# seungju-k1m/sac-td3-td7

Hardware: AMD Instinct MI355X
Metric: gradient-steps/sec (whole node), TD7 Humanoid-v4 batch=256 at 1/2/4/8 GPUs (higher is better)
Workload: dtype fp32

## Files before the change

### include/rle.h

```cpp
#ifndef RLE_H
#define RLE_H

#ifdef __cplusplus
extern "C" {
#endif

#define RLE_TD7 0
#define RLE_TD3 1
#define RLE_SAC 2

#define RLE_INFO_MAX 8

#define RLE_OK 0
#define RLE_EINVAL (-1)
#define RLE_EHIP (-2)
#define RLE_ESTATE (-3)

typedef struct rle_replay rle_replay;
typedef struct rle_engine rle_engine;

typedef struct rle_config {
  int algo;
  int state_dim, action_dim;
  int hidden;
  int batch;
  int use_lap;
  float discount;
  float policy_lr, critic_lr;
  float tau;
  float target_policy_noise, noise_clip;
  int policy_freq;
  int target_update_rate;
  float min_log_std, max_log_std;
  float tmp;
  unsigned long long seed;
  int device;
  int zs_dim;
  int n_hidden;
  int hidden_sizes[8];
  int act_actor, act_critic, act_encoder;
  float bc_lambda;
} rle_config;
typedef struct rle_config_ext {
  int size;
  float bc_alpha;
} rle_config_ext;
#define RLE_MAX_HIDDEN 6
#define RLE_ACT_DEFAULT 0
#define RLE_ACT_RELU 1
#define RLE_ACT_ELU 2
#define RLE_ACT_IDENTITY 3
#define RLE_ACT_LEAKY_RELU 4
#define RLE_ACT_SILU 5
#define RLE_ACT_GELU 6

#define RLE_FUSE_PRELAYER (1u << 0)
#define RLE_FUSE_PRE      (1u << 1)
#define RLE_FUSE_QDOT     (1u << 2)
#define RLE_FUSE_HEADDX   (1u << 3)
#define RLE_FUSE_NBDEFER  (1u << 4)
#define RLE_FUSE_SACFWD   (1u << 5)
#define RLE_FUSE_SACBWD   (1u << 6)
#define RLE_FUSE_FOLD     (1u << 7)
#define RLE_FUSE_PIPOLYAK (1u << 8)
#define RLE_FUSE_ENDSPLIT (1u << 9)
#define RLE_FUSE_PRIOSAMPLE (1u << 10)
#define RLE_FUSE_TWOSTAGE (1u << 11)
#define RLE_FUSE_SACPRE   (1u << 12)
#define RLE_FUSE_NORMFIN  (1u << 13)
#define RLE_FUSE_OPT_IN RLE_FUSE_PRIOSAMPLE
typedef struct rle_plan {
  int level_cap;
  int steps_per_graph;
  int pre_tn;
  int pl_tn;
  int tn_min;
  int flat_div;
  int balance;
  int tiny_w, uni_w, tiny_wg;
  int sched_cap;
  unsigned fuse_off;
  unsigned fuse_on;
  int rb;
  int pl_w;
  int lap_w, head_w, adam_w;
  int wide;
  int lpt;
  int dispatch;
  int dpf;
  int xcd;
} rle_plan;


int rle_replay_create(int device, long long capacity, int state_dim, int action_dim, int lap,
                      rle_replay** out);
int rle_replay_destroy(rle_replay* r);
int rle_replay_append(rle_replay* r, const float* state, const float* action, const float* reward,
                      const float* next_state, const float* notdone, long long count);
int rle_replay_state(rle_replay* r, long long* ptr, long long* size, float* max_priority);
int rle_replay_fill_random(rle_replay* r, long long count, unsigned long long seed);
int rle_replay_get_priority(rle_replay* r, float* out, long long n);
int rle_replay_set_priority(rle_replay* r, const float* p, long long n, float max_priority);
int rle_replay_sample_indices(rle_replay* r, int n, const float* u, long long* ind_out);
int rle_replay_update_priority(rle_replay* r, int n, const long long* ind, const float* p);
int rle_replay_reset_max_priority(rle_replay* r);
int rle_replay_gather(rle_replay* r, int n, const long long* ind, float* state, float* action,
                      float* reward, float* next_state, float* notdone);
int rle_replay_io_rows(void);
int rle_replay_export(rle_replay* r, long long first, long long count, float* state, float* action,
                      float* reward, float* next_state, float* notdone, float* priority);
int rle_replay_import(rle_replay* r, long long first, long long count, const float* state,
                      const float* action, const float* reward, const float* next_state,
                      const float* notdone, const float* priority);
int rle_replay_set_state(rle_replay* r, long long ptr, long long size, float max_priority);
int rle_replay_copy(rle_replay* dst, rle_replay* src);
int rle_replay_state_stats(rle_replay* r, float* mean, float* std);
int rle_replay_normalize_states(rle_replay* r, const float* shift, const float* scale);


int rle_create(const rle_config* cfg, rle_engine** out);
int rle_create_ext(const rle_config* cfg, const rle_config_ext* ext, rle_engine** out);
int rle_destroy(rle_engine* e);
// ... 67 lines not shown
```

### sac-td3-td7_amd/csrc/engine.cpp

```cpp
#include <hip/hip_runtime.h>
#include <hsa/hsa.h>
#include <hsa/hsa_ext_amd.h>
#include <hsa/hsa_ven_amd_loader.h>

#include <algorithm>
#include <atomic>
#include <chrono>
#include <cstdlib>
#include <cmath>
#include <cstdio>
#include <cstring>
#include <map>
#include <memory>
#include <mutex>
#include <stdexcept>
#include <string>
#include <thread>
#include <vector>

#include "ops.h"
#include "rle.h"

namespace rle {
hipError_t launch_level(const Op* d_ops, const Op* h_ops, int nops, int nwg, hipStream_t st,
// ... 233 lines not shown
  return 64;
}

static void check_gemm(const GemmArgs& g) {
  auto chk = [&](const Operand& o, bool xsplit, int xn) {
    REQUIRE(o.nseg >= 1 && o.nseg <= kMaxSeg, "gemm: bad segment count");
    for (int q = 0; q < o.nseg; ++q) {
      const Seg& s = o.seg[q];
      REQUIRE(s.p != nullptr && s.r0 % 16 == 0 && s.r1 > s.r0, "gemm: bad reduction segment");
      if (!xsplit) {
        REQUIRE(s.x0 == 0 && s.x1 >= xn, "gemm: segment must span the operand rows");
        if (q) REQUIRE(s.r0 == r16(o.seg[q - 1].r1), "gemm: reduction segments must be back to back");
      } else {
        REQUIRE(s.x0 % 16 == 0 && s.x1 % 16 == 0 && s.r0 == o.seg[0].r0 && s.r1 == o.seg[0].r1,
                "gemm: bad column split");
      }
    }
  };
  chk(g.A, false, g.M);
  chk(g.B, g.mode == GEMM_DW, g.N);
  if (g.mode == GEMM_DX || (g.mode == GEMM_FWD && g.B.nseg > 1)) {
    REQUIRE(g.B.nseg == g.A.nseg, "gemm: one W segment per A segment");
    for (int q = 0; q < g.A.nseg; ++q)
      REQUIRE(g.B.seg[q].r0 == g.A.seg[q].r0 && g.B.seg[q].r1 == g.A.seg[q].r1, "gemm: W / A segment mismatch");
  }
  REQUIRE(g.R <= 16 * 1024, "gemm: reduction too long");
}

static void xcd_plan(GemmArgs& g, bool xcd);

static bool gemm_variant_compiled(int vid, int ks = -1) {
#define RLE_VID(mode, epi, act, norm, pre, pk, sets) \
  (vid == gemm_vid(mode, epi, act, norm, pre) && (ks < 0 || ks_family(ks) == KS_EXT || (((sets) >> ks_family(ks)) & 1))) ||
  return RLE_GEMM_VARIANTS(RLE_VID) false;
#undef RLE_VID
}

static void gemm_finalize(GemmArgs& g, bool xcd = true) {
  int norm = 0;
  for (int q = 0; q < g.A.nseg; ++q) norm |= g.A.seg[q].norm.part != nullptr;
  for (int q = 0; q < g.B.nseg; ++q) norm |= g.B.seg[q].norm.part != nullptr;
  const int act_rt = g.mode == GEMM_FWD ? g.act : (g.mode == GEMM_DX ? g.dact : ACT_NONE);
  const int act = g.mode == GEMM_DW ? g.act : act_vslot(act_rt);
  REQUIRE(act_rt >= ACT_NONE && act_rt <= ACT_GELU, "gemm: activation");
  REQUIRE(act_rt <= ACT_TANH || ((g.has_pre == 0 || g.has_pre == 2) &&
                                 (g.epi == EPI_STORE || g.epi == EPI_QDOT || g.epi == EPI_QHEAD)),
          "gemm: LeakyReLU / SiLU / GELU run the plain and fused-loss-head paths only (kernels.hip kActRt)");
  REQUIRE(g.mode != GEMM_DX || !norm, "gemm: no DX variant with normed operands");
  REQUIRE(g.mode != GEMM_DW || g.epi == EPI_ADAM, "gemm: DW is always fused with Adam");
  REQUIRE(g.mode != GEMM_DW || act == ACT_NONE || (act == kDwGs && !norm && g.gscale) ||
              (act == kDwNb && !norm && g.nbx.t && g.nbm.part && g.nbdot && g.R <= 1024),
          "gemm: deferred AvgL1Norm backward / gradient scale operands");
  REQUIRE(g.mode != GEMM_DW || (act == kDwGs) == (g.gscale != nullptr), "gemm: gscale is the kDwGs variant's");
  REQUIRE(g.epi != EPI_NBDOT || (g.mode == GEMM_DX && act == ACT_NONE && g.nbx.t && g.norm_out),
          "gemm: EPI_NBDOT is a plain DX with x and partials");
  REQUIRE(g.epi != EPI_MSE || act == ACT_NONE, "gemm: MSE epilogue takes no activation");
  REQUIRE((g.dact == ACT_NONE) == (g.dsrc.t == nullptr) || g.mode != GEMM_DX, "gemm: DX derivative source");
  REQUIRE(g.has_pre != 1 || ((g.mode == GEMM_FWD || g.mode == GEMM_DX) && g.prea.N <= 32 && g.prea.seg < g.A.nseg &&
                               g.A.seg[g.prea.seg].r1 - g.A.seg[g.prea.seg].r0 <= 32 && g.prea.mode == g.mode &&
                               g.prea.R % 16 == 0),
          "gemm: pre-GEMM layout");
  {
    const HeadArgs& h = g.hd;
    const bool pol = h.mode == HEAD_MLP_POLICY;
    const bool modes = (h.mode == HEAD_TD7_LOSS && h.tgt_mode == HEAD_TD7_TARGET && h.vt && h.vmax_key && h.vmin_key) ||
                       (h.mode == HEAD_MLP_LOSS && h.tgt_mode == HEAD_MLP_TARGET && !h.vt) ||
                       (pol && h.tgt_mode < 0 && !h.lap && h.tp_n[0] == 0 && h.tp_n[1] == 0);
    const bool parts = h.qp[0] && h.qp[1] && h.qp_n[0] <= 64 && h.qp_n[1] <= 64 &&
                       (pol || (h.tp[0] && h.tp[1] && h.tp_n[0] <= 64 && h.tp_n[1] <= 64));
    REQUIRE(g.has_pre != 2 || (g.mode == GEMM_DX && g.epi == EPI_STORE && (act == ACT_ELU || act == ACT_RELU) &&
                               !norm && g.A.nseg == 1 && modes && parts && h.dact == act_rt && (!h.sac || h.logpi) &&
                               (!h.lap || h.prio) && h.H <= 256 && h.H % 4 == 0 && g.R == r16(h.H) &&
                               g.M % 16 == 0 && h.rows == h.nvalid && h.rows <= g.M && g.M - h.rows < 16 &&
                               (g.head_n == 0 || g.head_n == 1)),
            "gemm: fused loss head layout");
  }
  REQUIRE(g.epi != EPI_SACFWD || (g.mode == GEMM_FWD && act == ACT_NONE && !norm && g.has_pre == 0 && g.tn == 64 &&
                                   g.tiles_n == 1 && g.sf.A <= 32 && g.sf.ls_off + g.sf.A <= g.N && g.sf.eps.t &&
                                   g.sf.eps2.t && (g.sf.act.n || g.sf.act.t) && g.sf.logpi),
          "gemm: SAC actor forward epilogue operands");
  REQUIRE(g.epi != EPI_SACBWD || (g.mode == GEMM_DX && act == ACT_NONE && !norm && g.has_pre == 0 && g.sb.raw.t &&
                                   g.sb.eps2.t && (g.sb.dout.n || g.sb.dout.t) && g.sb.log_alpha &&
                                   g.sb.ls_off >= g.sb.mean_off + g.N),
          "gemm: SAC actor backward epilogue operands");
  REQUIRE((g.has_pre != 3 && g.has_pre != 4) || (((g.mode == GEMM_FWD && (g.epi == EPI_STORE || g.epi == EPI_QDOT) && g.prea.bias) ||
                                (g.mode == GEMM_DX && g.epi == EPI_STORE && g.prea.dsrc.t)) &&
                               act == ACT_RELU && !norm && g.A.nseg == 1 && g.prea.seg == 0 && g.prea.mode == g.mode &&
                               g.prea.act == ACT_RELU && g.prea.N == g.A.seg[0].r1 - g.A.seg[0].r0 && g.prea.N <= 256 &&
                               g.prea.N % 16 == 0 && g.prea.R % 16 == 0 && g.prea.R <= 48 && g.prea.B.nseg == 1 &&
                               g.R == g.prea.N &&
                               !g.pre.t && g.B.nseg == 1),
          "gemm: pre-layer layout");
  {
    const PreArgs& q = g.prea2;
    REQUIRE(g.has_pre != 4 || (g.mode == GEMM_FWD && g.epi == EPI_QDOT && q.mode == GEMM_FWD && q.N <= 32 &&
                               q.R % 16 == 0 && q.R <= 16 * 1024 && q.A.nseg == 1 && q.B.nseg == 1 &&
                               q.seg == 1 && g.prea.A.nseg == 2 && g.prea.A.seg[0].r0 == 0 &&
                               g.prea.A.seg[q.seg].r1 - g.prea.A.seg[q.seg].r0 <= 16 &&
                               g.prea.A.seg[q.seg].r0 % 16 == 0),
            "gemm: two-stage pre-layer layout");
  }
  {
    const PreArgs& q = g.prea;
    REQUIRE(g.has_pre != 5 || (g.mode == GEMM_FWD && g.epi == EPI_STORE && act == ACT_RELU && !norm &&
                               q.mode == GEMM_FWD && q.A.nseg == 1 && q.B.nseg == 1 && q.sac_a >= 1 &&
                               q.N == 2 * q.sac_a && q.N <= 48 && q.R % 16 == 0 && q.R <= 256 && q.bias &&
// ... 680 lines not shown
      const std::string what = a.what ? a.what : "";
      if (what.rfind("tape", 0) == 0) continue;
      const bool in_p = a.lo >= p0 && a.hi <= p1;
      if (!a.w || what == "adam w.t" || what == "adam bias") {
        if (op.kind == OP_GEMM && a.t >= 0) xr[(op.wg_begin + a.t) & 7].push_back({a.lo, a.hi});
        else once.push_back({a.lo, a.hi});
      }
      if (what.rfind("adam", 0) == 0) {
        if (a.w) t.adam_w += (double)(a.hi - a.lo);
        ad.push_back({a.lo, a.hi});
        if (what == "adam w.t" || what == "adam bias") ad.push_back({a.lo, a.hi});
      } else if (a.w) {
        aw.push_back({a.lo, a.hi});
      } else if (in_p) {
        wr.push_back({a.lo, a.hi});
      } else {
        ar.push_back({a.lo, a.hi});
      }
    }
  }
  t.act_r += union_bytes(ar);
  t.act_w += union_bytes(aw);
  t.w_r += union_bytes(wr);
  double adam = 0;
  for (auto& r : ad) adam += (double)(r.second - r.first);
  t.adam = adam;
  double xb = union_bytes(once);
  for (auto& r : xr) xb += union_bytes(r);
  t.xcd_r = xb;
  return t;
}

struct Prog {
  struct Item {
    std::vector<Op> ops;
    std::vector<int> rd, wr;
    int level = 0;
  };
  std::vector<Item> items;
  static constexpr int max_ops = kLevelOps;
  int rb = 0;
  int xcd = 1;
  std::map<const float*, std::pair<float*, int>> norm_fins;
  static bool rb_eligible(const GemmArgs& g) {
    bool seg_ok = true;
    for (int q = 0; q < g.B.nseg; ++q) seg_ok = seg_ok && g.B.seg[q].x0 % g.tn == 0;
    return g.mode == GEMM_DW && (g.tn == 32 || g.tn == 64) && g.has_pre == 0 && seg_ok;
  }
  void add(const Op& op, std::vector<int> rd, std::vector<int> wr) { add_group({op}, std::move(rd), std::move(wr)); }
  void add_group(std::vector<Op> ops, std::vector<int> rd, std::vector<int> wr) {
    for (Op& op : ops)
      if (op.kind == OP_GEMM) {
        op.gemm.hot.rb = rb && rb_eligible(op.gemm) ? 1 : 0;
        gemm_finalize(op.gemm, xcd != 0);
        check_gemm(op.gemm);
        if (std::getenv("RLE_AUDIT")) audit_gemm(op.gemm);
      }
    Item it;
    it.ops = std::move(ops);
    it.rd = std::move(rd);
    it.wr = std::move(wr);
    items.push_back(std::move(it));
  }
  int balance = 0;
  int tiny_w = 30, uni_w = 60, tiny_wg = 2;
  int pl_w = 0;
  int lap_w = 60, head_w = 60, adam_w = 8;
  int lpt = 0;
  int tiny_weight() const { return tiny_w ? tiny_w : 8; }
  int uniform_weight() const { return uni_w; }
  bool tiny_moves() const { return tiny_w != 0; }
  int op_weight(const Op& op) const {
    int x = 8;
    if (op.kind == OP_GEMM)
      x = op.gemm.R * op.gemm.tn / 1024 + (op.gemm.epi == EPI_ADAM ? adam_w : 0) + (op.gemm.has_pre >= 3 ? pl_w : 0);
    else if (op.kind == OP_HEAD) x = head_w;
    else if (op.kind == OP_SAMPLE_GATHER) x = op.sample.lap ? lap_w : uniform_weight();
    else if (op.kind == OP_STEP_END && op.end.mode != 1) x = tiny_weight();
    return x;
  }
  int item_weight(const Item& it) const {
    int w = 0;
    for (const Op& op : it.ops) w = std::max(w, op_weight(op));
    return w;
  }
  std::vector<std::vector<int>> successors() const {
    const int n = (int)items.size();
    std::vector<std::vector<int>> succ(n);
    std::map<int, int> lastw;
    std::map<int, std::vector<int>> readers;
    for (int i = 0; i < n; ++i) {
      const Item& it = items[i];
      auto edge = [&](int from) {
        if (from >= 0) succ[from].push_back(i);
      };
      for (int r : it.rd)
        if (r >= 0 && lastw.count(r)) edge(lastw[r]);
      for (int w : it.wr) {
        if (w < 0) continue;
        if (lastw.count(w)) edge(lastw[w]);
        for (int j : readers[w]) edge(j);
      }
      for (int w : it.wr)
        if (w >= 0) {
          lastw[w] = i;
          readers[w].clear();
// ... 1517 lines not shown
    g.A.seg[0] = seg_t(dz, 0, 0, Brows);
    g.A.nseg = 1;
    int koff = 0;
    for (size_t s = 0; s < X.size(); ++s) {
      const View& v = X[s];
      REQUIRE(v.cols == L.seg_p[s] && v.rows >= Brows && v.m.t, "dw: input view mismatch for " + L.wname);
      g.B.seg[s] = seg_t(v, koff, 0, Brows);
      if (v.norm && fused(RLE_FUSE_NORMFIN)) {
        const auto f = norm_fin(pg, v);
        g.B.seg[s].norm = f.first;
        rd.push_back(f.second);
      } else if (v.norm) {
        rd.push_back(v.norm_id);
      }
      rd.push_back(v.id);
      koff += L.seg_p[s];
    }
    g.B.nseg = (int)X.size();
    g.M = L.out;
    g.N = L.K;
    g.R = Brows;
    const auto tq = choose_tn(L.out, L.K);
    g.tn = tq.first;
    op.seq = tq.second;
    g.tiles_m = cdiv(L.out, kTileM);
    g.tiles_n = cdiv(L.K, g.tn) + 1;
    g.epi = EPI_ADAM;
    AdamArgs& ad = g.adam;
    ad.w = wmat(L);
    ad.b = bias(L);
    ad.mo = (long long)nP;
    ad.vo = 2LL * (long long)nP;
    ad.step = adam_step_of(asc_set) + cnt;
    ad.bc2s = adam_bc2s_of(asc_set) + cnt;
    ad.lr = lr;
    ad.beta1 = 0.9f;
    g.gscale = o.gscale;
    if (o.gscale) {
      REQUIRE(!nb_x, "dw: no gradient scale with a deferred AvgL1Norm backward");
      g.act = kDwGs;
      rd.push_back(o.gscale_id);
    }
    ad.beta2 = 0.999f;
    ad.omb1 = (float)(1.0 - 0.9);
    ad.omb2 = (float)(1.0 - 0.999);
    ad.eps = 1e-8f;
    ad.bias_col = cdiv(L.K, g.tn) * g.tn;
    ad.gsq = o.gsq;
    ad.gsq_b = o.gsq_b;
    ad.ptau = o.ptau;
    if (nb_x) {
      REQUIRE(dz.nbdot && nb_x->norm && nb_x->m.t && nb_x->rows >= Brows, "dw: deferred AvgL1Norm backward operands");
      g.act = kDwNb;
      g.nbx = nb_x->m;
      g.nbx_xs = nb_x->m.rbs;
      g.nbm = nb_x->nref();
      g.nbdot = dz.nbdot;
      g.nbdot_ld = dz.nbdot_ld;
      g.nbdot_n = dz.nbdot_n;
      rd.push_back(nb_x->id);
      if (fused(RLE_FUSE_NORMFIN)) {
        const auto f = norm_fin(pg, *nb_x);
        g.nbm = f.first;
        g.nb_width = nb_x->width;
        rd.push_back(f.second);
      } else {
        rd.push_back(nb_x->norm_id);
      }
      rd.push_back(dz.nbdot_id);
    }
    op.wg_count = g.tiles_m * g.tiles_n;
    pg.add(op, rd, wr);
  }

  bool pi_polyak_fused() const { return fused(RLE_FUSE_PIPOLYAK); }

  std::pair<NormRef, int> norm_fin(Prog& pg, const View& v) {
    REQUIRE(v.norm && v.norm_ld > 0, "norm_fin: not a normed view");
    auto it = pg.norm_fins.find(v.norm);
    if (it == pg.norm_fins.end()) {
      Op op{};
      op.kind = OP_NORMBWD;
      NormBwdArgs& a = op.nb;
      a.fwd = 2;
      a.rows = v.norm_ld;
      a.width = v.width;
      a.norm.part = v.norm;
      a.norm.ld = v.norm_ld;
      a.norm.row0 = 0;
      a.norm.nparts = v.nparts;
      a.norm.width = v.width;
      a.mout = mem.make<float>((size_t)v.norm_ld);
      op.wg_count = cdiv(v.norm_ld, kThreads);
      const int id = next_id++;
      pg.add(op, {v.norm_id}, {id});
      it = pg.norm_fins.emplace(v.norm, std::make_pair(a.mout, id)).first;
    }
    NormRef r{};
    r.part = it->second.first;
    r.ld = v.norm_ld;
    r.row0 = v.norm_row0;
    r.nparts = 1;
    r.width = 1;
    return {r, it->second.second};
  }

// ... 1208 lines not shown
  Graph capture(Prog& pg) {
    pg.balance = plan.balance;
    pg.tiny_w = plan.tiny_w;
    pg.uni_w = plan.uni_w;
    pg.tiny_wg = plan.tiny_wg;
    pg.pl_w = plan.pl_w;
    pg.lap_w = plan.lap_w;
    pg.head_w = plan.head_w;
    pg.adam_w = plan.adam_w;
    pg.lpt = plan.lpt;
    auto levels = pg.schedule(sched_cap());
    Graph G;
    size_t total = 0;
    for (auto& lv : levels) {
      G.nlaunch += (int)((lv.size() + kLevelOps - 1) / kLevelOps);
      G.off.push_back((int)total);
      G.nops.push_back((int)lv.size());
      int wg = 0;
      for (auto& op : lv) wg += op.wg_count;
      G.nwg.push_back(wg);
      total += lv.size();
    }
    static const char* kname[] = {"?", "gemm", "normbwd", "sreduce", "sgather", "head", "prio",
                                  "sacfwd", "sacbwd", "end", "polyak", "copy", "maxred", "ctrl", "noise",
                                  "foldbias", "bc"};
    static const bool traffic = [] {
      const char* e = std::getenv("RLE_TRAFFIC");
      return e && e[0] == '1';
    }();
    for (size_t l = 0; l < levels.size(); ++l) {
      G.desc += "L" + std::to_string(l) + " wg=" + std::to_string(G.nwg[l]) + ":";
      if (traffic) {
        const LevelTraffic t = level_traffic(levels[l], P, nP);
        char buf[220];
        snprintf(buf, sizeof buf, " [KB act_r %.0f act_w %.0f w_r %.0f adam %.0f other %.0f xcd_r %.0f adam_w %.0f]",
                 t.act_r / 1024, t.act_w / 1024, t.w_r / 1024, t.adam / 1024, t.other / 1024, t.xcd_r / 1024,
                 t.adam_w / 1024);
        G.desc += buf;
      }
      for (size_t k = 0; k < levels[l].size(); ++k) {
        const Op& op = levels[l][k];
        G.desc += std::string(" ") + (pg.crit_lv[l][k] ? "*" : "") + kname[op.kind];
        if (op.kind == OP_GEMM) {
          static const char* kepi[] = {"st", "adam", "mse", "qhead", "nbdot", "act", "qdot", "sacbwd", "sacfwd"};
          static_assert(sizeof(kepi) / sizeof(kepi[0]) == EPI_SACFWD + 1, "every epilogue has a name");
          const char* ep = op.gemm.mode == GEMM_DW && op.gemm.act == kDwNb ? "adam+nb"
                           : op.gemm.mode == GEMM_DW && op.gemm.act == kDwGs ? "adam+gs"
                           : op.gemm.has_pre == 2                         ? "head+dx"
                           : op.gemm.has_pre == 3                         ? (op.gemm.epi == EPI_QDOT ? "qdot+pl" : "st+pl")
                           : op.gemm.has_pre == 4                         ? "qdot+pl2"
                           : op.gemm.has_pre == 5                         ? "st+sacpre"
                                                                           : kepi[op.gemm.epi];
          G.desc += "[" + std::to_string(op.gemm.M) + "x" + std::to_string(op.gemm.N) + "x" +
                    std::to_string(op.gemm.R) + " " + ep + (op.gemm.hot.wide ? ".w" : "");
          const int art = op.gemm.mode == GEMM_FWD ? op.gemm.act : op.gemm.mode == GEMM_DX ? op.gemm.dact : ACT_NONE;
          if (art > ACT_TANH) G.desc += art == ACT_LEAKY ? " leaky" : art == ACT_SILU ? " silu" : " gelu";
          G.desc += "]";
        }
        if (std::getenv("RLE_DESC_WG")) G.desc += "/" + std::to_string(op.wg_count);
      }
      G.desc += "\n";
    }
    std::vector<Op> flat_ops;
    flat_ops.reserve(total);
    for (auto& lv : levels)
      for (auto& op : lv) {
        REQUIRE(op.kind != OP_GEMM || gemm_variant_compiled(op.gemm.vid, kernel_set()),
                "capture: a GEMM variant outside the engine's rle_level instance (ops.h RLE_GEMM_VARIANTS sets)");
        REQUIRE(kernel_set() == KS_ACT ||
                    ((op.kind != OP_GEMM || op.gemm.mode == GEMM_DW ||
                      (op.gemm.mode == GEMM_FWD ? op.gemm.act : op.gemm.dact) <= ACT_TANH) &&
                     (op.kind != OP_HEAD || op.head.dact <= ACT_TANH)),
                "capture: an activation of the KS_ACT rle_level instance in another instance's program");
        flat_ops.push_back(op);
      }
    G.d_ops = mem.make<Op>(total);
    HIPCHK(hipMemcpy(G.d_ops, flat_ops.data(), total * sizeof(Op), hipMemcpyHostToDevice));
    const char* tr_env = std::getenv("RLE_TRACE");
    if (tr_env && tr_env[0] == '1') {
      for (int w : G.nwg) G.trace_n += w;
      G.trace = mem.make<unsigned long long>((size_t)G.trace_n * trace_stride());
    }
    if (plan.dispatch == 1 && !G.trace) g_level_rec = &G.aql;
    HIPCHK(hipStreamBeginCapture(stream, hipStreamCaptureModeThreadLocal));
    long long tr_off = 0;
    const bool dpf = plan.dpf != 0;
    for (size_t l = 0; l < levels.size(); ++l) {
      const size_t ln = l + 1 < levels.size() ? l + 1 : 0;
      hipError_t e = launch_level(G.d_ops + G.off[l], levels[l].data(), G.nops[l], G.nwg[l], stream,
                                  G.trace ? G.trace + tr_off * trace_stride() : nullptr, G.d_ops + G.off[ln],
                                  dpf ? G.nops[ln] : 0, kernel_set());
      tr_off += G.nwg[l];
      if (e != hipSuccess) {
        g_level_rec = nullptr;
        hipGraph_t tmp;
        (void)hipStreamEndCapture(stream, &tmp);
        throw Error{RLE_EHIP, std::string("launch during capture: ") + hipGetErrorString(e)};
      }
    }
    g_level_rec = nullptr;
    HIPCHK(hipStreamEndCapture(stream, &G.g));
    if (!G.aql.empty()) {
      std::vector<unsigned char> ka(G.aql.size() * 128, 0);
      for (size_t i = 0; i < G.aql.size(); ++i) std::memcpy(ka.data() + i * 128, G.aql[i].ka, sizeof G.aql[i].ka);
      G.aql_ka = mem.make<unsigned char>(ka.size());
      HIPCHK(hipMemcpy(G.aql_ka, ka.data(), ka.size(), hipMemcpyHostToDevice));
    }
// ... 1763 lines not shown
```

### sac-td3-td7_amd/csrc/kernels.hip

```cpp
#include <hip/hip_runtime.h>
#include <math.h>
#include <stdint.h>

#include <cstring>
#include <type_traits>
#include <vector>

#include "ops.h"

#define CAS __attribute__((address_space(4)))
#define GAS __attribute__((address_space(1)))

namespace rle {

typedef float f32x4 __attribute__((ext_vector_type(4)));

template <class T>
__device__ __forceinline__ const GAS T* G(const T* p) {
  return (const GAS T*)p;
}
template <class T>
__device__ __forceinline__ GAS T* GW(T* p) {
  return (GAS T*)p;
}
// ... 402 lines not shown
      x[r] = bload(rx, vx + nx * 1024);
      if (!bias_ones) b[r] = bload(rb, vb + nx * 1024);
    }
  }
  return acc + acc1;
}

template <int RPT, int PM, int PD>
__device__ __forceinline__ void nb_tab_batched(const CAS GemmArgs& g, int n, float* ti, float* tg, float xw, int r0 = 0) {
  float sm[RPT], sd[RPT];
  row_sums<RPT, PM>(g.nbm.part, g.nbm.ld, g.nbm.row0 + r0, g.nbm.nparts, n, sm);
  row_sums<RPT, PD>(g.nbdot, g.nbdot_ld, r0, g.nbdot_n, n, sd);
#pragma unroll
  for (int r = 0; r < RPT; ++r) {
    const int i = threadIdx.x + r * kThreads;
    const float mean = sm[r] / (float)g.nbm.width, dot = sd[r] / 1.f;
    const bool clamped = mean < 1e-8f;
    const float inv = 1.f / (clamped ? 1e-8f : mean);
    if (i < n) {
      ti[i] = inv;
      tg[i] = clamped ? 0.f : (-dot * inv * inv) / xw;
    }
  }
}
__device__ __forceinline__ void build_nb_tab(const CAS GemmArgs& g, int n, float* ti, float* tg) {
  const float xw = (float)(g.nb_width ? g.nb_width : g.nbm.width);
  const int pm = g.nbm.nparts, pd = g.nbdot_n;
  if (n <= kThreads && pm <= 16 && pd <= 16) {
    nb_tab_batched<1, 16, 16>(g, n, ti, tg, xw);
    return;
  }
  if (n <= 4 * kThreads && pm == 1 && pd <= 8) {
    nb_tab_batched<4, 1, 8>(g, n, ti, tg, xw);
    return;
  }
  if (n <= 4 * kThreads && pm <= 4 && pd <= 4) {
    nb_tab_batched<4, 4, 4>(g, n, ti, tg, xw);
    return;
  }
  if (n <= 4 * kThreads && pm == 1 && pd <= 16) {
    nb_tab_batched<2, 1, 16>(g, min(n, 2 * kThreads), ti, tg, xw);
    if (n > 2 * kThreads) nb_tab_batched<2, 1, 16>(g, n - 2 * kThreads, ti + 2 * kThreads, tg + 2 * kThreads, xw, 2 * kThreads);
    return;
  }
#pragma unroll 1
  for (int i = threadIdx.x; i < n; i += kThreads) {
    const float mean = norm_mean_i(g.nbm.part, g.nbm.ld, i + g.nbm.row0, g.nbm.nparts, g.nbm.width);
    const float dot = norm_mean_i(g.nbdot, g.nbdot_ld, i, g.nbdot_n, 1);
    const bool clamped = mean < 1e-8f;
    const float inv = 1.f / (clamped ? 1e-8f : mean);
    ti[i] = inv;
    tg[i] = clamped ? 0.f : (-dot * inv * inv) / xw;
  }
}

__device__ __forceinline__ void chunk_loop2(__amdgpu_buffer_rsrc_t ra, int va, __amdgpu_buffer_rsrc_t rb, int vb0,
                                            int vb1, int n, f32x4& acc0, f32x4& acc1) {
  float4 a[kRing], b0[kRing], b1[kRing];
#pragma unroll
  for (int r = 0; r < kRing; ++r) {
    if (r >= n) break;
    a[r] = bload(ra, va + r * 1024);
    b0[r] = bload(rb, vb0 + r * 1024);
    b1[r] = bload(rb, vb1 + r * 1024);
  }
#pragma unroll 1
  for (int c = 0; c < n; c += kRing) {
#pragma unroll
    for (int r = 0; r < kRing; ++r) {
      if (c + r >= n) break;
      acc0 = mfma4(a[r], b0[r], acc0);
      acc1 = mfma4(a[r], b1[r], acc1);
      const int nx = c + r + kRing;
      if (nx >= n) continue;
      a[r] = bload(ra, va + nx * 1024);
      b0[r] = bload(rb, vb0 + nx * 1024);
      b1[r] = bload(rb, vb1 + nx * 1024);
    }
  }
}

constexpr int kRbOff = 2048;
template <int NB, int RG>
struct RbRing {
  float4 a[RG], x[RG], b[RG][NB];
};
template <int NB, int RG, bool NBX>
__device__ __forceinline__ void rb_issue(RbRing<NB, RG>& R, __amdgpu_buffer_rsrc_t ra, int va,
                                         __amdgpu_buffer_rsrc_t rbr, const int (&vbv)[NB], int nb, int n,
                                         __amdgpu_buffer_rsrc_t rx, int vx, bool bias_ones) {
  const float4 ones = make_float4(1.f, 1.f, 1.f, 1.f);
#pragma unroll
  for (int r = 0; r < RG; ++r) {
    if (r >= n) break;
    R.a[r] = bload(ra, va + r * 1024);
    if constexpr (NBX) R.x[r] = bload(rx, vx + r * 1024);
#pragma unroll
    for (int cb = 0; cb < NB; ++cb)
      if (cb < nb) R.b[r][cb] = bias_ones ? ones : bload(rbr, vbv[cb] + r * 1024);
  }
}
template <int NB, int RG, bool NBX>
__device__ __forceinline__ void rb_run(RbRing<NB, RG>& R, __amdgpu_buffer_rsrc_t ra, int va,
                                       __amdgpu_buffer_rsrc_t rbr, const int (&vbv)[NB], int nb, int n,
                                       f32x4 (&acc)[NB], const float* tabb, __amdgpu_buffer_rsrc_t rx, int vx,
                                       const float* ti, const float* tg, bool bias_ones) {
// ... 1062 lines not shown
      constexpr bool NBX = ACT == kDwNb;
      const int nq = (nch + 3) >> 2, q0 = wave * nq, q1 = min(nch, q0 + nq), nrun = max(0, q1 - q0);
      const int jc0 = jt * tn;
      int nb = 0;
#pragma unroll
      for (int cb = 0; cb < NB; ++cb) nb = jc0 + cb * 16 < gN ? cb + 1 : nb;
      if (bias_tile) nb = 1;
      int qb = 0;
#pragma unroll
      for (int q = 1; q < kMaxSeg; ++q)
        if (q < nseg_b && min(jc0, gN - 1) >= g.B.seg[q].x0) qb = q;
      const CAS Seg& sbq = g.B.seg[qb];
      int vbv[NB];
#pragma unroll
      for (int cb = 0; cb < NB; ++cb) vbv[cb] = ((((jc0 - sbq.x0) >> 4) + cb) * sbq.xs + q0) * 1024 + lb;
      const int va = ((i0 >> 4) * a0xs + q0) * 1024 + lb;
      const int vx = NBX ? ((i0 >> 4) * g.nbx_xs + q0) * 1024 + lb : 0;
      const auto rx = NBX ? rsrc(g.nbx.t) : rsrc(a0p);
      RbRing<NB, RG> R;
      rb_issue<NB, RG, NBX>(R, rsrc(a0p), va, rsrc(sbq.p), vbv, nb, nrun, rx, vx, bias_tile);
      const float* tabb = nullptr;
      if constexpr (NORM) {
        if (sbq.norm.part) build_norm_tab(sbq.norm, sbq.r1 - sbq.r0, tabs);
        __syncthreads();
        if (sbq.norm.part && !bias_tile) tabb = tabs + q0 * 16;
      }
      int tgo = 0;
      if constexpr (NBX) {
        tgo = (gR + 15) & ~15;
        build_nb_tab(g, gR, tabs, tabs + tgo);
        __syncthreads();
      }
      f32x4 ac[NB];
#pragma unroll
      for (int cb = 0; cb < NB; ++cb) ac[cb] = f32x4{0.f, 0.f, 0.f, 0.f};
      rb_run<NB, RG, NBX>(R, rsrc(a0p), va, rsrc(sbq.p), vbv, nb, nrun, ac, tabb, rx, vx, tabs + q0 * 16,
                          tabs + tgo + q0 * 16, bias_tile);
      acc = rb_exchange<NB>(ac, smem, cg, lead);
    };
    if (tn == 64) rbw(std::integral_constant<int, 4>{});
    else rbw(std::integral_constant<int, 2>{});
  } else {
    int qb = 0;
#pragma unroll
    for (int q = 1; q < kMaxSeg; ++q)
      if (q < nseg_b && j0 >= g.B.seg[q].x0) qb = q;
    const CAS Seg& sb = g.B.seg[qb];
    const bool run = active && c0 < c1;
    const int va = ((i0 >> 4) * a0xs + c0) * 1024 + lb;
    const int vb = (((j0 - sb.x0) >> 4) * sb.xs + c0) * 1024 + lb;
    const int vx = ACT == kDwNb ? ((i0 >> 4) * g.nbx_xs + c0) * 1024 + lb : 0;
    const int nrun = run ? c1 - c0 : 0;
    constexpr int RGD = ACT == kDwNb ? kRing : kRingDW;
    float4 ra[RGD], rb[RGD], rx[RGD];
    ring_issue<RGD>(ra, rb, rsrc(a0p), va, rsrc(sb.p), vb, nrun, bias_tile);
    if constexpr (ACT == kDwNb) {
#pragma unroll
      for (int r = 0; r < RGD; ++r)
        if (r < nrun) rx[r] = bload(rsrc(g.nbx.t), vx + r * 1024);
    }
    FINE_MARK(0);
    const float* tb = nullptr;
    if constexpr (NORM) {
      int off = 0, mine = -1;
      for (int q = 0; q < nseg_b; ++q) {
        const CAS Seg& s = g.B.seg[q];
        if (!s.norm.part) continue;
        build_norm_tab(s.norm, s.r1 - s.r0, tabs + off);
        if (q == qb) mine = off;
        off += (s.r1 - s.r0 + 15) & ~15;
      }
      __syncthreads();
      if (mine >= 0) tb = tabs + mine + c0 * 16;
    }
    int tgo = 0;
    if constexpr (ACT == kDwNb) {
      tgo = (gR + 15) & ~15;
      build_nb_tab(g, gR, tabs, tabs + tgo);
      __syncthreads();
    }
    FINE_MARK(1);
    if (run) {
      if constexpr (ACT == kDwNb) {
        acc = ring_run_nb<RGD>(ra, rx, rb, rsrc(a0p), va, rsrc(g.nbx.t), vx, rsrc(sb.p), vb, nrun, acc,
                               tabs + c0 * 16, tabs + tgo + c0 * 16, bias_tile);
      } else if (NORM && tb && !bias_tile)
        acc = ring_run<0, 2, RGD>(ra, rb, rsrc(a0p), va, rsrc(sb.p), vb, nrun, acc, 1.f, nullptr, tb, bias_tile);
      else
        acc = ring_run<0, 0, RGD>(ra, rb, rsrc(a0p), va, rsrc(sb.p), vb, nrun, acc, 1.f, nullptr, nullptr, bias_tile);
    }
  }
  trace_mark(tr, 2);
  if (ksl && !rbm) {
    if (!lead) *(f32x4*)(part + (wave * 64 + lane) * 4) = acc;
    __syncthreads();
    if (lead) {
      for (int q = 1; q < (1 << ksl); ++q) acc += *(const f32x4*)(part + ((wave + q) * 64 + lane) * 4);
    }
  }
  FINE_MARK(9);

  if constexpr (EPI == EPI_STORE || EPI == EPI_QDOT) {
    auto epi_store = [&](const f32x4 acc, const int i0, const int ib, const float4 ds, float* red) {
      float rowabs[4] = {0.f, 0.f, 0.f, 0.f};
      if (jok) {
        float y[4];
#pragma unroll
        for (int q = 0; q < 4; ++q) y[q] = acc[q] + pre_b;
        if constexpr (MODE == GEMM_FWD) {
          if (g.pre.t) mat_st4(g.pre, ib, j, make_float4(y[0], y[1], y[2], y[3]));
#pragma unroll
          for (int q = 0; q < 4; ++q) y[q] = act_f<ACT>(y[q], g.act);
          if constexpr (ACT == ACT_TANH) {
            if (g.noise.t && ib >= g.noise_row0) {
              const float4 e = mat_ld4(g.noise, ib - g.noise_row0, j);
              const float ev[4] = {e.x, e.y, e.z, e.w};
#pragma unroll
              for (int q = 0; q < 4; ++q) {
                const float nz = fminf(fmaxf(ev[q] * g.noise_sigma, -g.noise_clip), g.noise_clip);
                y[q] = fminf(fmaxf(y[q] + nz, -1.f), 1.f);
              }
            }
          }
        } else {
          const float dv[4] = {ds.x, ds.y, ds.z, ds.w};
#pragma unroll
          for (int q = 0; q < 4; ++q) y[q] *= act_b<ACT>(dv[q], g.dact);
        }
#pragma unroll
        for (int q = 0; q < 4; ++q) rowabs[q] = EPI == EPI_QDOT ? y[q] * qwj : fabsf(y[q]);
        mat_st4(g.out, ib, j, make_float4(y[0], y[1], y[2], y[3]));
      }
      if constexpr (MODE == GEMM_FWD) {
        if (EPI == EPI_QDOT || g.norm_out) {
#pragma unroll
// ... 1119 lines not shown
      d2 += d * d;
      GW(b.e.n)[nidx(b.e.cbn, r, j)] = c * d;
    }
    d2 = wg_sum(d2, smem);
    if (tid == 0) GW(b.part)[t] = d2;
    return;
  }
  if (BC3 && b.mode == 2) {
    float sa = 0.f;
    for (int i = tid; i < b.qp_n[0]; i += kThreads) sa += G(b.qp[0])[(size_t)i * b.qp_ld];
    const float q_abs = wg_sum(sa, smem) / (float)B;
    if (tid == 0) {
      GW(b.out)[0] = q_abs;
      GW(b.out)[1] = b.lambda / q_abs;
    }
    if (tid < A) GW(b.eye.t)[tidx(b.eye.rbs, tid, tid)] = q_abs / b.lambda;
    return;
  }
  const float b0 = G(b.qb[0])[0], b1 = G(b.qb[1])[0];
  float qa = 0.f;
  for (int r = tid; r < B; r += kThreads) {
    const float q0 = norm_mean_i(b.qp[0], b.qp_ld, r, b.qp_n[0], 1);
    const float q1 = norm_mean_i(b.qp[1], b.qp_ld, r, b.qp_n[1], 1);
    qa += BC3 && b.mode == 3 ? fabsf(fminf(q0 + b0, q1 + b1)) : fabsf(q0 + b0) + fabsf(q1 + b1);
  }
  if (BC3 && b.mode == 3) {
    const float q_abs = wg_sum(qa, smem) / (float)B;
    if (tid == 0) {
      GW(b.out)[0] = q_abs;
      GW(b.out)[1] = b.lambda / q_abs;
    }
    if (tid < A) GW(b.eye.t)[tidx(b.eye.rbs, tid, tid)] = q_abs / b.lambda;
    return;
  }
  const float q_abs = wg_sum(qa, smem) / (2.f * (float)B);
  if (tid == 0) GW(b.out)[0] = q_abs;
  if (tid < A) GW(b.eye.t)[tidx(b.eye.rbs, tid, tid)] = q_abs;
}


static_assert(kLevelOps == 12, "rle_level takes the op table as 12 scalar arguments");

template <bool TRACE, int KS>
#ifndef RLE_WAVES
#define RLE_WAVES 4
#endif
__global__ __launch_bounds__(kThreads, RLE_WAVES) void rle_level(unsigned e0, unsigned e1, unsigned e2, unsigned e3,
                                                                  unsigned e4, unsigned e5, unsigned e6, unsigned e7,
                                                                  unsigned e8, unsigned e9, unsigned e10, unsigned e11,
                                                                  const Op* ops_arg, unsigned long long* trace_arg,
                                                                  const Op* next_arg, unsigned next_lines) {
  constexpr int kSmemF = (KS == KS_TD7W || ks_family(KS) == KS_EXT) && kWideSmem > 6144 ? kWideSmem : 6144;
  static_assert(kSmemF >= kRbOff + 4096, "LDS for the register-blocked exchange");
  __shared__ __attribute__((aligned(16))) float smem[kSmemF];
  const unsigned long long t_in = TRACE ? __builtin_amdgcn_s_memrealtime() : 0ull;
  if ((e0 >> 31) && blockIdx.x < 8) {
    const unsigned nl = next_lines;
    const char* nb = (const char*)next_arg;
    unsigned v0 = 0, v1 = 0;
    const unsigned l0 = threadIdx.x, l1 = threadIdx.x + kThreads;
    if (l0 < nl) asm volatile("global_load_dword %0, %1, off" : "=v"(v0) : "v"(nb + l0 * 64) : "memory");
    if (l1 < nl) asm volatile("global_load_dword %0, %1, off" : "=v"(v1) : "v"(nb + l1 * 64) : "memory");
    asm volatile("s_waitcnt vmcnt(0)" ::"v"(v0), "v"(v1) : "memory");
    return;
  }
  const unsigned entry[kLevelOps] = {e0 & 0x7fffffffu, e1, e2, e3, e4, e5, e6, e7, e8, e9, e10, e11};
  const int wg = (int)blockIdx.x - (int)(e0 >> 31) * 8;
  int k = 0;
  unsigned e = entry[0];
#pragma unroll
  for (int q = 1; q < kLevelOps; ++q) {
    const unsigned x = entry[q];
    const bool in = (int)(x & 0xffffu) <= wg;
    e = in ? x : e;
    k = in ? q : k;
  }
  const int kind = (e >> 16) & 0xf, vid = e >> 20;
  const CAS Op* ops = (const CAS Op*)ops_arg;
  const int wb = (int)(e & 0xffffu);
  const CAS Op& op = ops[k];
  const int t = wg - wb;
  unsigned long long* tr = TRACE ? trace_arg + (size_t)wg * kTraceStride : nullptr;
  if (TRACE && threadIdx.x == 0) tr[0] = t_in;
  if (kind != OP_GEMM) {
    unsigned dsink;
    asm volatile(
        "s_load_dword %0, %1, 0x0\n\t"
        "s_load_dword %0, %1, 0x40\n\t"
        "s_load_dword %0, %1, 0x80\n\t"
        "s_load_dword %0, %1, 0xc0\n\t"
        "s_load_dword %0, %1, 0x100\n\t"
        "s_load_dword %0, %1, 0x140\n\t"
        "s_load_dword %0, %1, 0x180\n\t"
        "s_load_dword %0, %1, 0x1c0\n\t"
        "s_waitcnt lgkmcnt(0)"
        : "=&s"(dsink)
        : "s"(&op));
    (void)dsink;
  }
  FINE_MARK(7);
  switch (kind) {
#define RLE_OP(K, call)                       \
  case K:                                     \
    asm volatile("; op case " #K ::);         \
    call;                                     \
    break;
// ... 599 lines not shown
```

### sac-td3-td7_amd/csrc/ops.h

```cpp
#pragma once
#include <stdint.h>

namespace rle {

constexpr int kThreads = 256;
constexpr int kTileM = 16;
constexpr int kTileN = 64;
constexpr int kMaxSeg = 4;
constexpr int kInfoMax = 8;
constexpr int kMaxHidden = 6;
constexpr int kGsqT = 2 * (kMaxHidden + 1);

enum OpKind : int {
  OP_GEMM = 1,
  OP_NORMBWD = 2,
  OP_SAMPLE_REDUCE = 3,
  OP_SAMPLE_GATHER = 4,
  OP_HEAD = 5,
  OP_PRIORITY = 6,
  OP_SAC_ACTOR = 7,
  OP_SAC_ACTOR_BWD = 8,
  OP_STEP_END = 9,
  OP_POLYAK = 10,
  OP_COPY = 11,
// ... 94 lines not shown
  X(GEMM_FWD, EPI_MSE, ACT_NONE, 1, 0, 0, 1)        \
  X(GEMM_FWD, EPI_ACT, ACT_TANH, 0, 0, 0, 3)        \
  X(GEMM_FWD, EPI_QDOT, ACT_ELU, 0, 0, 0, 1)        \
  X(GEMM_FWD, EPI_QDOT, ACT_RELU, 0, 0, 0, 2)       \
  X(GEMM_FWD, EPI_QDOT, ACT_NONE, 0, 0, 0, 0)       \
  X(GEMM_DX, EPI_STORE, ACT_NONE, 0, 0, 0, 3)       \
  X(GEMM_DX, EPI_STORE, ACT_RELU, 0, 0, 0, 3)       \
  X(GEMM_DX, EPI_STORE, ACT_ELU, 0, 0, 0, 3)        \
  X(GEMM_DX, EPI_STORE, ACT_TANH, 0, 0, 0, 3)       \
  X(GEMM_DX, EPI_NBDOT, ACT_NONE, 0, 0, 0, 1)       \
  X(GEMM_DW, EPI_ADAM, ACT_NONE, 0, 0, 0, 3)        \
  X(GEMM_DW, EPI_ADAM, ACT_NONE, 1, 0, 0, 1)        \
  X(GEMM_DW, EPI_ADAM, kDwNb, 0, 0, 0, 1)           \
  X(GEMM_DW, EPI_ADAM, kDwGs, 0, 0, 0, 0)           \
  X(GEMM_FWD, EPI_STORE, ACT_NONE, 0, 1, 1, 1)      \
  X(GEMM_FWD, EPI_STORE, ACT_RELU, 0, 1, 1, 3)      \
  X(GEMM_FWD, EPI_STORE, ACT_ELU, 1, 1, 1, 1)       \
  X(GEMM_DX, EPI_STORE, ACT_RELU, 0, 1, 1, 3)       \
  X(GEMM_DX, EPI_SACBWD, ACT_NONE, 0, 0, 0, 2)      \
  X(GEMM_FWD, EPI_SACFWD, ACT_NONE, 0, 0, 0, 2)     \
  X(GEMM_DX, EPI_STORE, ACT_ELU, 0, 2, 2, 1)        \
  X(GEMM_DX, EPI_STORE, ACT_RELU, 0, 2, 2, 2)       \
  X(GEMM_FWD, EPI_STORE, ACT_RELU, 0, 3, 3, 2)      \
  X(GEMM_FWD, EPI_QDOT, ACT_RELU, 0, 3, 3, 2)       \
  X(GEMM_DX, EPI_STORE, ACT_RELU, 0, 3, 3, 2)       \
  X(GEMM_FWD, EPI_QDOT, ACT_RELU, 1, 3, 4, 2)       \
  X(GEMM_FWD, EPI_STORE, ACT_RELU, 1, 1, 5, 2)
constexpr bool wide_variant(int mode, int epi, int pk) {
  return pk == 0 && mode != 2  &&
         (epi == EPI_STORE || epi == EPI_QDOT || epi == EPI_MSE || epi == EPI_QHEAD || epi == EPI_NBDOT);
}
enum KernelSet : int { KS_TD7 = 0, KS_MLP = 1, KS_EXT = 2, KS_TD7W = 3, KS_ACT = 4, KS_COUNT = 5 };
constexpr int ks_family(int ks) { return ks == KS_TD7W ? KS_TD7 : ks == KS_ACT ? KS_EXT : ks; }

enum GemmMode : int {
  GEMM_FWD = 0,
  GEMM_DX = 1,
  GEMM_DW = 2,
};

struct GemmHot {
  int ks_log, tiles_n, tn, N, R;
  float inv_tiles_n;
  int bias_col, nseg_a, nseg_b;
  int a0xs, a0r0, a0r1, b0xs, tiles;
  const float* a0p;
  const float* b0p;
  const float* bias;
  int xb, tmb;
  float inv_tmb, inv_xb, inv_blast;
  int nfull;
  int rb;
  int wide;
  int pad_[4];
};
static_assert(sizeof(GemmHot) == 128, "GemmHot is loaded as 2 x 16 dwords");

__host__ __device__ inline void xcd_tile(int t, int T, int tiles_n, int xb, int tmb, int nfull, float inv_tmb,
                                         float inv_xb, float inv_blast, int& it, int& jt) {
  const int q = T >> 3, m = T & 7, r0 = t & 7;
  const int p = r0 * q + (r0 < m ? r0 : m) + (t >> 3);
  const int band = (int)(((float)p + 0.5f) * inv_tmb);
  const int rem = p - band * tmb;
  const bool full = band < nfull;
  const int bw = full ? xb : tiles_n - nfull * xb;
  it = (int)(((float)rem + 0.5f) * (full ? inv_xb : inv_blast));
  jt = band * xb + rem - it * bw;
}

struct PreArgs {
  Operand A, B;
  int mode;
  int N, R;
  int seg;
  int act;
  int sac_a;
  const float* bias;
  Mat noise; float noise_sigma, noise_clip;
  Mat dsrc;
};

enum HeadMode : int {
  HEAD_TD7_TARGET = 0,
  HEAD_TD7_LOSS = 1,
  HEAD_TD7_POLICY = 2,
  HEAD_MLP_TARGET = 3,
  HEAD_MLP_LOSS = 4,
  HEAD_MLP_POLICY = 5,
};

struct HeadArgs {
  int mode, rows, H, lap;
  Mat h[2];
  Mat dsrc[2];
  int dact;
  int nvalid;
  const float* w[2];
  int w_cbn;
  const float* b[2];
  const float* reward; const float* notdone;
  float* y;
  Mat dz[2];
  Mat dq[2];
  float* loss_part;
  float* prio;
  float gamma;
  int sac;
  int alpha_lin;
  const float* logpi;
// ... 362 lines not shown
```

### sac-td3-td7_amd/rl/_engine.py

```python

from __future__ import annotations

import contextlib
import ctypes
import os
import threading

import numpy as np

RLE_TD7, RLE_TD3, RLE_SAC = 0, 1, 2
RLE_EVAL_Q, RLE_EVAL_ZS, RLE_EVAL_ZSA = 0, 1, 2
INFO_MAX = 8
REPLAY_IO_ROWS = 8192

_HERE = os.path.dirname(os.path.abspath(__file__))
LIB_PATH = os.environ.get("RLE_LIB") or os.path.join(os.path.dirname(_HERE), "lib", "librle.so")

_lib = None

_f32p = ctypes.POINTER(ctypes.c_float)
_i64p = ctypes.POINTER(ctypes.c_longlong)
_vp = ctypes.c_void_p
_cs = ctypes.c_char_p
_int = ctypes.c_int
_ll = ctypes.c_longlong


class Config(ctypes.Structure):

    _fields_ = [
        ("algo", _int), ("state_dim", _int), ("action_dim", _int), ("hidden", _int),
        ("batch", _int), ("use_lap", _int), ("discount", ctypes.c_float),
        ("policy_lr", ctypes.c_float), ("critic_lr", ctypes.c_float), ("tau", ctypes.c_float),
        ("target_policy_noise", ctypes.c_float), ("noise_clip", ctypes.c_float),
        ("policy_freq", _int), ("target_update_rate", _int), ("min_log_std", ctypes.c_float),
        ("max_log_std", ctypes.c_float), ("tmp", ctypes.c_float), ("seed", ctypes.c_ulonglong),
        ("device", _int), ("zs_dim", _int), ("n_hidden", _int), ("hidden_sizes", _int * 8),
        ("act_actor", _int), ("act_critic", _int), ("act_encoder", _int),
        ("bc_lambda", ctypes.c_float),
    ]


class ConfigExt(ctypes.Structure):

    _fields_ = [("size", _int), ("bc_alpha", ctypes.c_float)]


def make_config_ext(bc_alpha=0.0) -> ConfigExt:
    return ConfigExt(ctypes.sizeof(ConfigExt), float(bc_alpha))


ACT_CODES = {"default": 0, "relu": 1, "elu": 2, "identity": 3, "leaky_relu": 4, "silu": 5, "gelu": 6}


class Plan(ctypes.Structure):

    _fields_ = [
        ("level_cap", _int), ("steps_per_graph", _int), ("pre_tn", _int), ("pl_tn", _int), ("tn_min", _int),
        ("flat_div", _int), ("balance", _int), ("tiny_w", _int), ("uni_w", _int), ("tiny_wg", _int),
        ("sched_cap", _int), ("fuse_off", ctypes.c_uint), ("fuse_on", ctypes.c_uint), ("rb", _int),
        ("pl_w", _int), ("lap_w", _int), ("head_w", _int), ("adam_w", _int), ("wide", _int), ("lpt", _int),
        ("dispatch", _int), ("dpf", _int), ("xcd", _int),
    ]


FUSE = {"prelayer": 1 << 0, "pre": 1 << 1, "qdot": 1 << 2, "headdx": 1 << 3, "nbdefer": 1 << 4, "sacfwd": 1 << 5,
        "sacbwd": 1 << 6, "fold": 1 << 7, "pipolyak": 1 << 8, "endsplit": 1 << 9, "priosample": 1 << 10,
        "twostage": 1 << 11, "sacpre": 1 << 12, "normfin": 1 << 13}


def make_plan(fuse_off=(), fuse_on=(), **kw) -> Plan:
    p = Plan()
    _check(lib().rle_plan_default(ctypes.byref(p)))
    for k, v in kw.items():
        if k not in dict(Plan._fields_):
            raise ValueError(f"unknown plan field {k!r}")
        setattr(p, k, int(v))
    def bits(names):
        b = 0
        for name in ([names] if isinstance(names, str) else names):
            b |= FUSE[name]
        return b

    p.fuse_off, p.fuse_on = bits(fuse_off), bits(fuse_on)
    return p


def parse_plan(text: str) -> Plan:
    kw, off, on = {}, (), ()
    for item in filter(None, (t.strip() for t in (text or "").split(","))):
        k, _, v = item.partition("=")
        if k == "fuse_off":
            off = tuple(filter(None, v.split("+")))
        elif k == "fuse_on":
            on = tuple(filter(None, v.split("+")))
        else:
            kw[k] = int(v)
    return make_plan(off, on, **kw)


def plan_dict(p: Plan) -> dict:
    d = {k: getattr(p, k) for k, _ in Plan._fields_}
    d["fuse_off"] = [n for n, b in FUSE.items() if p.fuse_off & b]
    d["fuse_on"] = [n for n, b in FUSE.items() if p.fuse_on & b]
    return d


STATE_PARAMS, STATE_ADAM_M, STATE_ADAM_V, STATE_ALL = 1, 2, 4, 7

_scratch = np.empty(0, np.float32)
_scratch_lock = threading.Lock()


@contextlib.contextmanager
def state_scratch(n):
    global _scratch
    with _scratch_lock:
        if _scratch.size < n:
            _scratch = np.empty(n, np.float32)
        yield _scratch[:n]

# ... 489 lines not shown
```

Before: 8330.

## Stage AvgL1Norm-backward strip in LDS for kDwNb weight-gradient GEMMs

Adds a staged path for the deferred AvgL1Norm-backward weight-gradient GEMM. Each wave computes a share of the normalized-gradient rows and writes them into a shared LDS strip, then after a barrier all waves run MFMAs from that strip. Previously each wave recomputed the transform from its own global loads. The path is gated by a new fuse bit and by an LDS-fit check on R. It keeps per-element fused/unfused FMA ordering so results stay bitwise identical, at the cost of an added block barrier and LDS traffic.

```diff
diff --git a/include/rle.h b/include/rle.h
--- a/include/rle.h
+++ b/include/rle.h
@@ -68,6 +68,7 @@
 #define RLE_FUSE_TWOSTAGE (1u << 11)
 #define RLE_FUSE_SACPRE   (1u << 12)
 #define RLE_FUSE_NORMFIN  (1u << 13)
+#define RLE_FUSE_NBSTAGE  (1u << 14)
 #define RLE_FUSE_OPT_IN RLE_FUSE_PRIOSAMPLE
 typedef struct rle_plan {
   int level_cap;
diff --git a/sac-td3-td7_amd/csrc/engine.cpp b/sac-td3-td7_amd/csrc/engine.cpp
--- a/sac-td3-td7_amd/csrc/engine.cpp
+++ b/sac-td3-td7_amd/csrc/engine.cpp
@@ -309,6 +309,9 @@
               (act == kDwNb && !norm && g.nbx.t && g.nbm.part && g.nbdot && g.R <= 1024),
           "gemm: deferred AvgL1Norm backward / gradient scale operands");
   REQUIRE(g.mode != GEMM_DW || (act == kDwGs) == (g.gscale != nullptr), "gemm: gscale is the kDwGs variant's");
+  REQUIRE(!g.hot.nbst || (g.mode == GEMM_DW && act == kDwNb && !g.hot.rb && !g.hot.wide && nb_stage_fits(g.R)),
+          "gemm: the staged AvgL1Norm-backward strip is the kDwNb variant's and fits the level's LDS "
+          "(ops.h nb_stage_fits)");
   REQUIRE(g.epi != EPI_NBDOT || (g.mode == GEMM_DX && act == ACT_NONE && g.nbx.t && g.norm_out),
           "gemm: EPI_NBDOT is a plain DX with x and partials");
   REQUIRE(g.epi != EPI_MSE || act == ACT_NONE, "gemm: MSE epilogue takes no activation");
@@ -1095,6 +1098,7 @@
     for (Op& op : ops)
       if (op.kind == OP_GEMM) {
         op.gemm.hot.rb = rb && rb_eligible(op.gemm) ? 1 : 0;
+        if (op.gemm.hot.rb) op.gemm.hot.nbst = 0;
         gemm_finalize(op.gemm, xcd != 0);
         check_gemm(op.gemm);
         if (std::getenv("RLE_AUDIT")) audit_gemm(op.gemm);
@@ -2718,6 +2722,7 @@
     if (nb_x) {
       REQUIRE(dz.nbdot && nb_x->norm && nb_x->m.t && nb_x->rows >= Brows, "dw: deferred AvgL1Norm backward operands");
       g.act = kDwNb;
+      g.hot.nbst = fused(RLE_FUSE_NBSTAGE) && nb_stage_fits(g.R) && kernel_set() == KS_TD7 ? 1 : 0;
       g.nbx = nb_x->m;
       g.nbx_xs = nb_x->m.rbs;
       g.nbm = nb_x->nref();
@@ -4032,7 +4037,8 @@
                            : op.gemm.has_pre == 5                         ? "st+sacpre"
                                                                            : kepi[op.gemm.epi];
           G.desc += "[" + std::to_string(op.gemm.M) + "x" + std::to_string(op.gemm.N) + "x" +
-                    std::to_string(op.gemm.R) + " " + ep + (op.gemm.hot.wide ? ".w" : "");
+                    std::to_string(op.gemm.R) + " " + ep + (op.gemm.hot.wide ? ".w" : "") +
+                    (op.gemm.hot.nbst ? ".s" : "");
           const int art = op.gemm.mode == GEMM_FWD ? op.gemm.act : op.gemm.mode == GEMM_DX ? op.gemm.dact : ACT_NONE;
           if (art > ACT_TANH) G.desc += art == ACT_LEAKY ? " leaky" : art == ACT_SILU ? " silu" : " gelu";
           G.desc += "]";
diff --git a/sac-td3-td7_amd/csrc/kernels.hip b/sac-td3-td7_amd/csrc/kernels.hip
--- a/sac-td3-td7_amd/csrc/kernels.hip
+++ b/sac-td3-td7_amd/csrc/kernels.hip
@@ -478,6 +478,82 @@
     ti[i] = inv;
     tg[i] = clamped ? 0.f : (-dot * inv * inv) / xw;
   }
+}
+
+__device__ __forceinline__ float nb_fused(float a, float iv, float x, float gv) {
+  return __builtin_fmaf(a, iv, sgnf(x) * gv);
+}
+__device__ __forceinline__ float nb_unfused(float a, float iv, float x, float gv) {
+#pragma clang fp contract(off)
+  const float p = a * iv, q = sgnf(x) * gv;
+  return p + q;
+}
+template <int RG = kRing>
+__device__ __forceinline__ void nb_stage_issue(float4 (&a)[RG], float4 (&x)[RG], float4 (&b)[RG],
+                                               __amdgpu_buffer_rsrc_t rg, int va, __amdgpu_buffer_rsrc_t rx, int vx,
+                                               int s, int q1, __amdgpu_buffer_rsrc_t rb, int vb, int n, bool bias_ones) {
+#pragma unroll
+  for (int r = 0; r < RG; ++r) {
+    if (r >= n) break;
+    b[r] = bias_ones ? make_float4(1.f, 1.f, 1.f, 1.f) : bload(rb, vb + r * 1024);
+  }
+#pragma unroll
+  for (int r = 0; r < RG; ++r) {
+    if (s + r >= q1) break;
+    a[r] = bload(rg, va + (s + r) * 1024);
+    x[r] = bload(rx, vx + (s + r) * 1024);
+  }
+}
+template <int RG = kRing>
+__device__ __forceinline__ f32x4 nb_stage_run(float4 (&sg)[RG], float4 (&sx)[RG], float4 (&b)[RG],
+                                              __amdgpu_buffer_rsrc_t rg, int va, __amdgpu_buffer_rsrc_t rx, int vx,
+                                              int q0, int q1, __amdgpu_buffer_rsrc_t rb, int vb, int c0, int per, int n,
+                                              f32x4 acc, const float* ti, const float* tg, float* strip,
+                                              bool bias_ones) {
+  static_assert(RG == 4, "the slot of a chunk in ring_run_nb's ring");
+  const int lane = threadIdx.x & 63, rl = (lane >> 4) << 2;
+#pragma unroll 1
+  for (int s = q0; s < q1; s += RG) {
+    if (s != q0) {
+#pragma unroll
+      for (int r = 0; r < RG; ++r) {
+        if (s + r >= q1) break;
+        sg[r] = bload(rg, va + (s + r) * 1024);
+        sx[r] = bload(rx, vx + (s + r) * 1024);
+      }
+    }
+#pragma unroll
+    for (int r = 0; r < RG; ++r) {
+      const int k = s + r;
+      if (k >= q1) break;
+      const float4 iv = *(const float4*)(ti + k * 16 + rl), gv = *(const float4*)(tg + k * 16 + rl);
+      float4 y;
+      if (((k - k / per * per) & 3) == 3)
+        y = make_float4(nb_unfused(sg[r].x, iv.x, sx[r].x, gv.x), nb_unfused(sg[r].y, iv.y, sx[r].y, gv.y),
+                        nb_unfused(sg[r].z, iv.z, sx[r].z, gv.z), nb_unfused(sg[r].w, iv.w, sx[r].w, gv.w));
+      else
+        y = make_float4(nb_fused(sg[r].x, iv.x, sx[r].x, gv.x), nb_fused(sg[r].y, iv.y, sx[r].y, gv.y),
+                        nb_fused(sg[r].z, iv.z, sx[r].z, gv.z), nb_fused(sg[r].w, iv.w, sx[r].w, gv.w));
+      *(float4*)(strip + k * 256 + lane * 4) = y;
+    }
+  }
+  __syncthreads();
+  const float* la = strip + c0 * 256 + lane * 4;
+  f32x4 acc1 = {0.f, 0.f, 0.f, 0.f};
+#pragma unroll 1
+  for (int c = 0; c < n; c += RG) {
+#pragma unroll
+    for (int r = 0; r < RG; ++r) {
+      if (c + r >= n) break;
+      const float4 y = *(const float4*)(la + (c + r) * 256);
+      if (r & 1) acc1 = mfma4(y, b[r], acc1);
+      else acc = mfma4(y, b[r], acc);
+      const int nx = c + r + RG;
+      if (nx >= n) continue;
+      if (!bias_ones) b[r] = bload(rb, vb + nx * 1024);
+    }
+  }
+  return acc + acc1;
 }
 
 __device__ __forceinline__ void chunk_loop2(__amdgpu_buffer_rsrc_t ra, int va, __amdgpu_buffer_rsrc_t rb, int vb0,
@@ -1646,12 +1722,20 @@
     const int vx = ACT == kDwNb ? ((i0 >> 4) * g.nbx_xs + c0) * 1024 + lb : 0;
     const int nrun = run ? c1 - c0 : 0;
     constexpr int RGD = ACT == kDwNb ? kRing : kRingDW;
+    bool nbst = false;
+    if constexpr (ACT == kDwNb && !EXT && !WIDE) nbst = h1[12] != 0;
     float4 ra[RGD], rb[RGD], rx[RGD];
-    ring_issue<RGD>(ra, rb, rsrc(a0p), va, rsrc(sb.p), vb, nrun, bias_tile);
-    if constexpr (ACT == kDwNb) {
-#pragma unroll
-      for (int r = 0; r < RGD; ++r)
-        if (r < nrun) rx[r] = bload(rsrc(g.nbx.t), vx + r * 1024);
+    const int snq = (nch + 3) >> 2, sq0 = wave * snq, sq1 = min(nch, sq0 + snq);
+    const int sva = (i0 >> 4) * a0xs * 1024 + lb, svx = ACT == kDwNb ? (i0 >> 4) * g.nbx_xs * 1024 + lb : 0;
+    if (nbst) {
+      nb_stage_issue<RGD>(ra, rx, rb, rsrc(a0p), sva, rsrc(g.nbx.t), svx, sq0, sq1, rsrc(sb.p), vb, nrun, bias_tile);
+    } else {
+      ring_issue<RGD>(ra, rb, rsrc(a0p), va, rsrc(sb.p), vb, nrun, bias_tile);
+      if constexpr (ACT == kDwNb) {
+#pragma unroll
+        for (int r = 0; r < RGD; ++r)
+          if (r < nrun) rx[r] = bload(rsrc(g.nbx.t), vx + r * 1024);
+      }
     }
     FINE_MARK(0);
     const float* tb = nullptr;
@@ -1674,7 +1758,10 @@
       __syncthreads();
     }
     FINE_MARK(1);
-    if (run) {
+    if (nbst) {
+      acc = nb_stage_run<RGD>(ra, rx, rb, rsrc(a0p), sva, rsrc(g.nbx.t), svx, sq0, sq1, rsrc(sb.p), vb, c0, per, nrun, acc,
+                              tabs, tabs + tgo, tabs + 2 * tgo, bias_tile);
+    } else if (run) {
       if constexpr (ACT == kDwNb) {
         acc = ring_run_nb<RGD>(ra, rx, rb, rsrc(a0p), va, rsrc(g.nbx.t), vx, rsrc(sb.p), vb, nrun, acc,
                                tabs + c0 * 16, tabs + tgo + c0 * 16, bias_tile);
@@ -2900,6 +2987,7 @@
                                                                   const Op* next_arg, unsigned next_lines) {
   constexpr int kSmemF = (KS == KS_TD7W || ks_family(KS) == KS_EXT) && kWideSmem > 6144 ? kWideSmem : 6144;
   static_assert(kSmemF >= kRbOff + 4096, "LDS for the register-blocked exchange");
+  static_assert(kSmemF >= kLevelSmemF, "LDS for the staged kDwNb strip (ops.h nb_stage_fits)");
   __shared__ __attribute__((aligned(16))) float smem[kSmemF];
   const unsigned long long t_in = TRACE ? __builtin_amdgcn_s_memrealtime() : 0ull;
   if ((e0 >> 31) && blockIdx.x < 8) {
diff --git a/sac-td3-td7_amd/csrc/ops.h b/sac-td3-td7_amd/csrc/ops.h
--- a/sac-td3-td7_amd/csrc/ops.h
+++ b/sac-td3-td7_amd/csrc/ops.h
@@ -170,9 +170,15 @@
   int nfull;
   int rb;
   int wide;
-  int pad_[4];
+  int nbst;
+  int pad_[3];
 };
 static_assert(sizeof(GemmHot) == 128, "GemmHot is loaded as 2 x 16 dwords");
+
+constexpr int kLevelSmemF = 6144;
+constexpr int nb_stage_floats(int R) { return 64 + 1024 + 2 * ((R + 15) & ~15) + 16 * R; }
+constexpr bool nb_stage_fits(int R) { return nb_stage_floats(R) <= kLevelSmemF; }
+static_assert(nb_stage_fits(256) && !nb_stage_fits(1024), "the flagship's strip fits; B = 1024 keeps the per-wave path");
 
 __host__ __device__ inline void xcd_tile(int t, int T, int tiles_n, int xb, int tmb, int nfull, float inv_tmb,
                                          float inv_xb, float inv_blast, int& it, int& jt) {
diff --git a/sac-td3-td7_amd/rl/_engine.py b/sac-td3-td7_amd/rl/_engine.py
--- a/sac-td3-td7_amd/rl/_engine.py
+++ b/sac-td3-td7_amd/rl/_engine.py
@@ -66,7 +66,7 @@
 
 FUSE = {"prelayer": 1 << 0, "pre": 1 << 1, "qdot": 1 << 2, "headdx": 1 << 3, "nbdefer": 1 << 4, "sacfwd": 1 << 5,
         "sacbwd": 1 << 6, "fold": 1 << 7, "pipolyak": 1 << 8, "endsplit": 1 << 9, "priosample": 1 << 10,
-        "twostage": 1 << 11, "sacpre": 1 << 12, "normfin": 1 << 13}
+        "twostage": 1 << 11, "sacpre": 1 << 12, "normfin": 1 << 13, "nbstage": 1 << 14}
 
 
 def make_plan(fuse_off=(), fuse_on=(), **kw) -> Plan:
```

Result: no change. 8355 (median of 3 runs) (+0.3%).
